# shroglck/open-pi-zero

Measured on AMD Instinct MI355X. Metric: train samples/sec at gbsz 1024 (bf16 fwd+bwd+clip+AdamW), higher is better.
Workload: dtype bf16; 1 GPU; Pi0 bridge training step: 256 img + 20 text + 1 proprio + 4 action tokens; model=pi0 (SigLIP-So400m/14 + Gemma-2B + 0.3B action expert), global_batch=1024, micro_batch=256, grad_accum=4, seq_len=281, parallelism=dp1

## Files before the change

open-pi-zero_amd/csrc/pz_flash.hip:

```cpp
#include "pz_common.h"

#include <type_traits>

namespace {

constexpr int FA_KB = 64;
constexpr int FA_NW = 4;
constexpr int FA_QS = 32;

template <int HD>
struct FaDims {
  static constexpr int HDK = (HD + 31) / 32 * 32;
  static constexpr int HDV = (HD + 15) / 16 * 16;
  static constexpr int NKS = HDK / 32;
  static constexpr int NDB = HDV / 16;
  static constexpr int ROW = HD == 256 ? 272 : (HD == 72 ? 112 : HDK + 16);
  static constexpr int FNW = HD == 256 ? 8 : 4;
  static constexpr int FNQB = HD == 256 ? 1 : 2;
};

__device__ __forceinline__ bool fa_allowed(int64_t i, int64_t j, int64_t cnt, int64_t P, int64_t C) {
  if (i < P) return i < cnt && j < cnt;
  if (i < P + C) return j < cnt || (j >= P && j < P + C);
  return j < cnt || j >= P;
// ... 697 lines not shown
    crow[qb] = mk.dead(t) ? 0.f : ff.crow_live;
  }
  f32x4 dq[D::NDB][2];
#pragma unroll
  for (int db = 0; db < D::NDB; ++db) dq[db][0] = dq[db][1] = f32x4{0.f, 0.f, 0.f, 0.f};

  __syncthreads();
  stk.store(Ks2[0]);
  stv.store(Vs2[0]);
  __syncthreads();
  for (int kb = 0; kb < nkb; ++kb) {
    const bf16_t* Ks = Ks2[kb & 1];
    const bf16_t* Vs = Vs2[kb & 1];
    const bool more = kb + 1 < nkb;
    if (more) {
      stk.load(K, a.ldk, (int64_t)(kb + 1) * JQ_KB, a.nk);
      stv.load(V, a.ldv, (int64_t)(kb + 1) * JQ_KB, a.nk);
    }
    const bool full = (kb + 1) * JQ_KB <= full_keys;
    f32x4 ds[2][2];
#pragma unroll
    for (int i = 0; i < 2; ++i) {
      bf16x8 kfr[D::NKS], vfr[D::NKS];
#pragma unroll
      for (int ks = 0; ks < D::NKS; ++ks) {
        kfr[ks] = frag_row<D::ROW>(Ks, i * 16, ks * 32, lane);
        vfr[ks] = frag_row<D::ROW>(Vs, i * 16, ks * 32, lane);
      }
#pragma unroll
      for (int qb = 0; qb < 2; ++qb) {
        f32x4 sv = {0.f, 0.f, 0.f, 0.f}, dp = {0.f, 0.f, 0.f, 0.f};
#pragma unroll
        for (int ks = 0; ks < D::NKS; ++ks) {
          sv = mfma(kfr[ks], qf[qb][ks], sv);
          dp = mfma(vfr[ks], df[qb][ks], dp);
        }
#pragma unroll
        for (int e = 0; e < 4; ++e) {
          const bool ok = full || ((rb[qb] >> fa_key_class(mk, kb * JQ_KB + i * 16 + 4 * g + e)) & 1);
          float pe, dse;
          ff.eval<CAP>(sv[e], dp[e], lse2[qb], crow[qb], del[qb], ok, pe, dse);
          ds[i][qb][e] = dse;
        }
      }
    }
    const bf16x8 sb0 = pack8(ds[0][0], ds[1][0]), sb1 = pack8(ds[0][1], ds[1][1]);
    constexpr int HB = (D::NDB + 1) / 2;
#pragma unroll
    for (int hb = 0; hb < 2; ++hb) {
      bf16x8 kt[HB];
#pragma unroll
      for (int x = 0; x < HB; ++x)
        if (hb * HB + x < D::NDB) kt[x] = frag_tr<D::ROW>(Ks, 0, (hb * HB + x) * 16, lane);
#pragma unroll
      for (int x = 0; x < HB; ++x) {
        const int db = hb * HB + x;
        if (db < D::NDB) {
          dq[db][0] = mfma(kt[x], sb0, dq[db][0]);
          dq[db][1] = mfma(kt[x], sb1, dq[db][1]);
        }
      }
    }
    if (more) {
      stk.store(Ks2[(kb + 1) & 1]);
      stv.store(Vs2[(kb + 1) & 1]);
    }
    __syncthreads();
  }
#pragma unroll
  for (int qb = 0; qb < 2; ++qb) {
    const int64_t r = (int64_t)qblk * RPW + wave * 32 + qb * 16 + (lane & 15);
    if (r >= a.nq) continue;
    bf16_t* dQ = (bf16_t*)a.dq + b * a.q_bstride + h * a.q_hstride + r * a.ldq;
#pragma unroll
    for (int db = 0; db < D::NDB; ++db) {
      const int d = db * 16 + 4 * g;
      if (d < HD)
        *reinterpret_cast<u32x2*>(dQ + d) = u32x2{pack2bf(dq[db][qb][0] * ff.scale, dq[db][qb][1] * ff.scale),
                                                  pack2bf(dq[db][qb][2] * ff.scale, dq[db][qb][3] * ff.scale)};
    }
  }
}

constexpr int JP_NW = 8, JP_MAXKB = 5;

constexpr int FR_MAX = 256, FR_NW = 8;

template <int HD>
__global__ void __launch_bounds__(FR_NW * 64) flash_fwd_res_kernel(pz_flash_args a) {
  using D = FaDims<HD>;
  constexpr int NT = FR_NW * 64;
  extern __shared__ __attribute__((aligned(16))) char fa_smem[];
  bf16_t* Kall = reinterpret_cast<bf16_t*>(fa_smem);
  bf16_t* Vall = Kall + FR_MAX * D::ROW;
  const int lane = threadIdx.x & 63, wave = threadIdx.x >> 6, g = lane >> 4;
  int64_t zh;
  int qblk;
  fa_unit_block((int)((a.nq + FR_NW * 16 - 1) / (FR_NW * 16)), (int)(a.Z * a.H), zh, qblk);
  const int64_t b = zh / a.H, h = zh % a.H;
  const int64_t q0 = (int64_t)qblk * (FR_NW * 16) + wave * 16;
  const bf16_t* Q = (const bf16_t*)a.q + b * a.q_bstride + h * a.q_hstride;
  const bf16_t* K = (const bf16_t*)a.k + b * a.k_bstride + h * a.k_hstride;
  const bf16_t* V = (const bf16_t*)a.v + b * a.v_bstride + h * a.v_hstride;
  const FaMask mk(a, b);
  {
    TileStager<HD, D::ROW, FR_MAX, NT> stk, stv;
    stk.load(K, a.ldk, 0, a.nk);
    stv.load(V, a.ldv, 0, a.nk);
    zero_pad_cols<HD, D::HDK, D::ROW, FR_MAX, NT>(Kall);
    zero_pad_cols<HD, D::HDK, D::ROW, FR_MAX, NT>(Vall);
    stk.store(Kall);
    stv.store(Vall);
  }
  bf16x8 qf[D::NKS];
  const int64_t rq = q0 + (lane & 15);
#pragma unroll
  for (int ks = 0; ks < D::NKS; ++ks) {
    const int c = ks * 32 + 8 * g;
    qf[ks] = (rq < a.nq && c < HD) ? *reinterpret_cast<const bf16x8*>(Q + rq * a.ldq + c) : bf16x8{};
  }
  f32x4 o[D::NDB];
#pragma unroll
  for (int db = 0; db < D::NDB; ++db) o[db] = f32x4{0.f, 0.f, 0.f, 0.f};
  float m = -INFINITY, l = 0.f;
  const int t = mk.token((int)rq);
  const int nkb = (int)((a.nk + FA_KB - 1) / FA_KB);
  __syncthreads();
  for (int kb = 0; kb < nkb; ++kb) {
    const bf16_t* Ks = Kall + kb * FA_KB * D::ROW;
    const bf16_t* Vs = Vall + kb * FA_KB * D::ROW;
    f32x4 sc[4];
#pragma unroll
    for (int i = 0; i < 4; ++i) sc[i] = f32x4{0.f, 0.f, 0.f, 0.f};
#pragma unroll
    for (int ks = 0; ks < D::NKS; ++ks)
#pragma unroll
      for (int i = 0; i < 4; ++i) sc[i] = mfma(frag_row<D::ROW>(Ks, i * 16, ks * 32, lane), qf[ks], sc[i]);
    float mx = -INFINITY;
#pragma unroll
    for (int i = 0; i < 4; ++i)
#pragma unroll
      for (int e = 0; e < 4; ++e) {
        const float x = fa_logit(mk, sc[i][e], t, kb * FA_KB + i * 16 + 4 * g + e);
        sc[i][e] = x;
        mx = fmaxf(mx, x);
      }
    mx = fmaxf(mx, __shfl_xor(mx, 16, 64));
    mx = fmaxf(mx, __shfl_xor(mx, 32, 64));
    const float mn = fmaxf(m, mx);
    const float alpha = mn == -INFINITY ? 1.f : __expf(m - mn);
    float sum = 0.f;
#pragma unroll
    for (int i = 0; i < 4; ++i)
#pragma unroll
      for (int e = 0; e < 4; ++e) {
        const float pv = mn == -INFINITY ? 0.f : __expf(sc[i][e] - mn);
        sc[i][e] = pv;
        sum += pv;
      }
    sum += __shfl_xor(sum, 16, 64);
    sum += __shfl_xor(sum, 32, 64);
    l = l * alpha + sum;
    m = mn;
#pragma unroll
    for (int db = 0; db < D::NDB; ++db) o[db] *= alpha;
    const bf16x8 pf0 = pack8(sc[0], sc[1]), pf1 = pack8(sc[2], sc[3]);
#pragma unroll
// ... 1206 lines not shown
          f32x4 sv = {0.f, 0.f, 0.f, 0.f}, dp = {0.f, 0.f, 0.f, 0.f};
#pragma unroll
          for (int ks = 0; ks < 3; ++ks) {
            sv = mfma(qa[ks], kfr[kb2][ks], sv);
            dp = mfma(da[ks], vfr[kb2][ks], dp);
          }
          float pe[4], de[4];
#pragma unroll
          for (int e = 0; e < 4; ++e) {
            pe[e] = __builtin_amdgcn_exp2f(fmaf(sv[e], sl2, -l2r[e]));
            de[e] = pe[e] * (dp[e] - dlr[e]);
          }
          pp[i][kb2][0] = pack2bf(pe[0], pe[1]);
          pp[i][kb2][1] = pack2bf(pe[2], pe[3]);
          dd[i][kb2][0] = pack2bf(de[0], de[1]);
          dd[i][kb2][1] = pack2bf(de[2], de[3]);
        }
      }
      if (last && un < units) issue_kv(un);
      auto cat4 = [](unsigned x0, unsigned x1, unsigned x2, unsigned x3) {
        return __builtin_bit_cast(bf16x8, u32x4{x0, x1, x2, x3});
      };
      const bf16x8 pb0 = cat4(pp[0][0][0], pp[0][0][1], pp[1][0][0], pp[1][0][1]);
      const bf16x8 pb1 = cat4(pp[0][1][0], pp[0][1][1], pp[1][1][0], pp[1][1][1]);
      const bf16x8 sb0 = cat4(dd[0][0][0], dd[0][0][1], dd[1][0][0], dd[1][0][1]);
      const bf16x8 sb1 = cat4(dd[0][1][0], dd[0][1][1], dd[1][1][0], dd[1][1][1]);
      const unsigned da0 = fs_lds_addr(Ds + (4 * g + ((lane & 15) >> 2)) * FS_ROW + 4 * (lane & 3));
      const unsigned qa0 = fs_lds_addr(Qs + (4 * g + ((lane & 15) >> 2)) * FS_ROW + 4 * (lane & 3));
      s16x4 td[5][2], tq[5][2];
#define FS_TR(db, hf)                                             \
  td[db][hf] = fs_tr<(16 * (hf)) * FS_ROW * 2 + (db) * 32>(da0); \
  tq[db][hf] = fs_tr<(16 * (hf)) * FS_ROW * 2 + (db) * 32>(qa0)
#define FS_MM(db)                                                                \
  {                                                                              \
    const bf16x8 dt = fs_cat(td[db][0], td[db][1]), qt = fs_cat(tq[db][0], tq[db][1]); \
    dv[db][0] = mfma(dt, pb0, dv[db][0]);                                        \
    dv[db][1] = mfma(dt, pb1, dv[db][1]);                                        \
    dk[db][0] = mfma(qt, sb0, dk[db][0]);                                        \
    dk[db][1] = mfma(qt, sb1, dk[db][1]);                                        \
  }
      FS_TR(0, 0); FS_TR(0, 1); FS_TR(1, 0); FS_TR(1, 1);
      asm volatile("s_waitcnt lgkmcnt(0)"
                   : "+v"(td[0][0]), "+v"(td[0][1]), "+v"(td[1][0]), "+v"(td[1][1]), "+v"(tq[0][0]), "+v"(tq[0][1]),
                     "+v"(tq[1][0]), "+v"(tq[1][1]));
      FS_TR(2, 0); FS_TR(2, 1); FS_TR(3, 0); FS_TR(3, 1);
      FS_MM(0) FS_MM(1)
      asm volatile("s_waitcnt lgkmcnt(0)"
                   : "+v"(td[2][0]), "+v"(td[2][1]), "+v"(td[3][0]), "+v"(td[3][1]), "+v"(tq[2][0]), "+v"(tq[2][1]),
                     "+v"(tq[3][0]), "+v"(tq[3][1]));
      FS_TR(4, 0); FS_TR(4, 1);
      FS_MM(2) FS_MM(3)
      asm volatile("s_waitcnt lgkmcnt(0)" : "+v"(td[4][0]), "+v"(td[4][1]), "+v"(tq[4][0]), "+v"(tq[4][1]));
      FS_MM(4)
#undef FS_MM
#undef FS_TR
    };
#pragma unroll 1
    for (int qs = 0; qs < FS_N / FA_QS - 1; ++qs) step(qs, false);
    step(FS_N / FA_QS - 1, true);
    FS_WAIT_VM(0);
#pragma unroll
    for (int kb2 = 0; kb2 < 2; ++kb2) {
      const int key = wave * 32 + kb2 * 16 + (lane & 15);
      bf16_t* dK = (bf16_t*)a.dk + b * a.k_bstride + h * a.k_hstride + (int64_t)key * a.ldk;
      bf16_t* dV = (bf16_t*)a.dv + b * a.v_bstride + h * a.v_hstride + (int64_t)key * a.ldv;
#pragma unroll
      for (int db = 0; db < 5; ++db) {
        const int d = db * 16 + 4 * g;
        if (d < 72) {
          *reinterpret_cast<u32x2*>(dK + d) = u32x2{pack2bf(dk[db][kb2][0] * a.scale, dk[db][kb2][1] * a.scale),
                                                    pack2bf(dk[db][kb2][2] * a.scale, dk[db][kb2][3] * a.scale)};
          *reinterpret_cast<u32x2*>(dV + d) =
              u32x2{pack2bf(dv[db][kb2][0], dv[db][kb2][1]), pack2bf(dv[db][kb2][2], dv[db][kb2][3])};
        }
      }
    }
    if (un < units && w0) tix.publish(tk, fa_smem + ((t + 1) & 1) * 2 * FS_IMG + FS_SLOT1);
    FS_BARRIER();
    u = un;
  }
}

constexpr int JD_SLOT = 64 * 512, JD_SMEM = 4 * JD_SLOT;

struct JdDma {
  int wave, lane;
  bool trs;
  __device__ __forceinline__ JdDma(int wave_, int lane_, bool trs_) : wave(wave_), lane(lane_), trs(trs_) {}
  __device__ __forceinline__ void issue(const bf16_t* X, int64_t ld, int kb, int nk, char* slot, int) const {
    int ln = lane;
    asm volatile("" : "+v"(ln));
#pragma unroll
    for (int s = 0; s < 4; ++s) {
      const int r = 2 * (wave * 4 + s) + (ln >> 5), pch = ln & 31;
      const int coff = 8 * (pch ^ (trs ? 2 * (r & 7) : (r & 15)));
      int key = kb * 64 + r;
      key = key < nk ? key : nk - 1;
      fs_glds16(X + (int64_t)key * ld + coff, slot + (wave * 4 + s) * 1024);
    }
  }
};

template <int K2, int DG>
__device__ __forceinline__ void jd_pv_group(f32x4 (&o)[16], const unsigned (&vs)[8], const bf16x8& pk) {
  s16x4 tv[4][2];
#define JD_TR(u, hf) tv[u][hf] = fs_tr<(K2 * 32 + 16 * (hf)) * 512 + ((DG * 4 + (u)) & 8) * 32>(vs[(DG * 4 + (u)) & 7])
  JD_TR(0, 0); JD_TR(0, 1); JD_TR(1, 0); JD_TR(1, 1); JD_TR(2, 0); JD_TR(2, 1); JD_TR(3, 0); JD_TR(3, 1);
#undef JD_TR
  asm volatile("s_waitcnt lgkmcnt(0)"
               : "+v"(tv[0][0]), "+v"(tv[0][1]), "+v"(tv[1][0]), "+v"(tv[1][1]), "+v"(tv[2][0]), "+v"(tv[2][1]),
                 "+v"(tv[3][0]), "+v"(tv[3][1]));
#pragma unroll
  for (int u = 0; u < 4; ++u) o[DG * 4 + u] = mfma(fs_cat(tv[u][0], tv[u][1]), pk, o[DG * 4 + u]);
}

template <bool CAP>
__global__ void __launch_bounds__(JP_NW * 64, 1) flash_fwd_probs_dma_kernel(pz_flash_args a, bf16_t* P, bf16_t* TC,
                                                                         int64_t ldp) {
  extern __shared__ __attribute__((aligned(16))) char fa_smem[];
  constexpr int RPW = JP_NW * 16;
  const int lane = threadIdx.x & 63, wave = threadIdx.x >> 6, g = lane >> 4, l15 = lane & 15;
  int64_t zh;
  int qblk;
  fa_unit_block((int)((a.nq + RPW - 1) / RPW), (int)(a.Z * a.H), zh, qblk);
  const int64_t b = zh / a.H, h = zh % a.H;
  const int64_t r = (int64_t)qblk * RPW + wave * 16 + l15;
  const bool live = r < a.nq;
  const bf16_t* Q = (const bf16_t*)a.q + b * a.q_bstride + h * a.q_hstride;
  const bf16_t* K = (const bf16_t*)a.k + b * a.k_bstride + h * a.k_hstride;
  const bf16_t* V = (const bf16_t*)a.v + b * a.v_bstride + h * a.v_hstride;
  const FaMask mk(a, b);
  const FaFast ff(a);
  const int nk = (int)a.nk;
  const JdDma dmk(wave, lane, false), dmv(wave, lane, true);
  bf16x8 qf[8];
  {
    const bf16_t* qrow = Q + (live ? r : 0) * a.ldq + 8 * g;
#define JD_QLD(ks) asm volatile("global_load_dwordx4 %0, %1, off offset:%2" : "=v"(qf[ks]) : "v"(qrow), "i"((ks) * 64) : "memory")
    JD_QLD(0); JD_QLD(1); JD_QLD(2); JD_QLD(3); JD_QLD(4); JD_QLD(5); JD_QLD(6); JD_QLD(7);
#undef JD_QLD
  }
  auto issue = [&](int s) {
    char* slot = fa_smem + (s % 4) * JD_SLOT;
    if (s < 5) dmk.issue(K, a.ldk, s, nk, slot, wave);
    else dmv.issue(V, a.ldv, s - 5, nk, slot, wave);
  };
  issue(0);
  issue(1);
  issue(2);
  const int t = mk.token((int)r);
  const bool dead = mk.dead(t);
  const int rb = fa_row_bits(mk, t), full_keys = fa_full_keys(mk);
  const bool clean = __ballot(dead || !live) == 0ull;
  f32x4 sc[JP_MAXKB][4];
  u32x2 tcv[JP_MAXKB][4];
  float mx = -INFINITY;
  auto logits_blk = [&](int kb) {
    auto logits = [&](auto FAST) {
#pragma unroll
      for (int i = 0; i < 4; ++i) {
        float tv[4];
#pragma unroll
        for (int e = 0; e < 4; ++e) {
          const float sv = sc[kb][i][e];
          float th = 0.f, x2;
          if constexpr (CAP) {
            th = fmaf(-2.f, __builtin_amdgcn_rcpf(__builtin_amdgcn_exp2f(sv * ff.k2) + 1.f), 1.f);
            x2 = th * ff.crow_live;
          } else {
            x2 = sv * ff.crow_live;
          }
          if constexpr (!decltype(FAST)::value) {
            const int j = kb * FA_KB + i * 16 + 4 * g + e;
            const bool ok = j < nk && (j < full_keys || ((rb >> fa_key_class(mk, j)) & 1));
            x2 = ok ? x2 : -INFINITY;
            th = (dead || j >= nk) ? 0.f : th;
          }
          sc[kb][i][e] = x2;
          mx = fmaxf(mx, x2);
          tv[e] = th;
        }
        tcv[kb][i] = u32x2{pack2bf(tv[0], tv[1]), pack2bf(tv[2], tv[3])};
      }
    };
    if (clean && (kb + 1) * 64 <= full_keys) logits(std::true_type{});
    else logits(std::false_type{});
  };
#pragma unroll
  for (int kb = 0; kb < JP_MAXKB; ++kb) {
    FS_WAIT_VM(8);
    FS_BARRIER();
    if (kb == 0)
      asm volatile("" : "+v"(qf[0]), "+v"(qf[1]), "+v"(qf[2]), "+v"(qf[3]), "+v"(qf[4]), "+v"(qf[5]), "+v"(qf[6]),
                   "+v"(qf[7]));
    issue(kb + 3);
    const char* slot = fa_smem + (kb % 4) * JD_SLOT + l15 * 512;
#pragma unroll
    for (int i = 0; i < 4; ++i) sc[kb][i] = f32x4{0.f, 0.f, 0.f, 0.f};
#pragma unroll
    for (int ks = 0; ks < 8; ++ks) {
      const char* kp = slot + 16 * ((4 * ks + g) ^ l15);
#pragma unroll
      for (int i = 0; i < 4; ++i) sc[kb][i] = mfma(*reinterpret_cast<const bf16x8*>(kp + i * 8192), qf[ks], sc[kb][i]);
    }
    if (kb >= 1) logits_blk(kb - 1);
  }
  logits_blk(JP_MAXKB - 1);
  FS_WAIT_VM(4);
  bf16_t* prow = P + (b * a.nq + (live ? r : 0)) * ldp;
  if (TC) {
    bf16_t* trow = TC + (b * a.nq + (live ? r : 0)) * ldp;
#pragma unroll
    for (int kb = 0; kb < JP_MAXKB; ++kb)
#pragma unroll
      for (int i = 0; i < 4; ++i) {
        const int j0 = kb * FA_KB + i * 16 + 4 * g;
        if (clean && (kb + 1) * 64 <= full_keys) *reinterpret_cast<u32x2*>(trow + j0) = tcv[kb][i];
// ... 2 lines not shown
  }
  mx = fs_max4(mx);
  float sum = 0.f;
#pragma unroll
  for (int kb = 0; kb < JP_MAXKB; ++kb)
#pragma unroll
    for (int i = 0; i < 4; ++i)
#pragma unroll
      for (int e = 0; e < 4; ++e) {
        const float pv = __builtin_amdgcn_exp2f(sc[kb][i][e] - mx);
        sc[kb][i][e] = pv;
        sum += pv;
      }
  sum = fs_sum4(sum);
  const float inv = 1.f / sum, uni = 1.f / (float)nk;
  bf16x8 pf[JP_MAXKB][2];
#pragma unroll
  for (int kb = 0; kb < JP_MAXKB; ++kb) {
    unsigned pk[4][2];
    auto probs = [&](auto FAST) {
#pragma unroll
      for (int i = 0; i < 4; ++i) {
        if constexpr (decltype(FAST)::value) {
          pk[i][0] = pack2bf(sc[kb][i][0] * inv, sc[kb][i][1] * inv);
          pk[i][1] = pack2bf(sc[kb][i][2] * inv, sc[kb][i][3] * inv);
        } else {
          float pv[4];
#pragma unroll
          for (int e = 0; e < 4; ++e) {
            const int j = kb * FA_KB + i * 16 + 4 * g + e;
            pv[e] = dead ? (j < nk ? uni : 0.f) : sc[kb][i][e] * inv;
          }
          pk[i][0] = pack2bf(pv[0], pv[1]);
          pk[i][1] = pack2bf(pv[2], pv[3]);
        }
        const int j0 = kb * FA_KB + i * 16 + 4 * g;
        if (decltype(FAST)::value || (live && j0 < ldp)) *reinterpret_cast<u32x2*>(prow + j0) = u32x2{pk[i][0], pk[i][1]};
      }
    };
    if (clean && (kb + 1) * 64 <= full_keys) probs(std::true_type{});
    else probs(std::false_type{});
    pf[kb][0] = __builtin_bit_cast(bf16x8, u32x4{pk[0][0], pk[0][1], pk[1][0], pk[1][1]});
    pf[kb][1] = __builtin_bit_cast(bf16x8, u32x4{pk[2][0], pk[2][1], pk[3][0], pk[3][1]});
  }
  f32x4 o[16];
#pragma unroll
  for (int db = 0; db < 16; ++db) o[db] = f32x4{0.f, 0.f, 0.f, 0.f};
  const int q4 = l15 >> 2, p4 = lane & 3, w = 4 * (g & 1) + q4;
  unsigned va[8];
#pragma unroll
  for (int d7 = 0; d7 < 8; ++d7) va[d7] = fs_lds_addr(fa_smem + (4 * g + q4) * 512 + 32 * (d7 ^ w) + 8 * p4);
#pragma unroll
  for (int kb = 0; kb < JP_MAXKB; ++kb) {
    const int s = 5 + kb;
    if (s == 7) FS_WAIT_VM(8);
    if (s == 8) FS_WAIT_VM(4);
    if (s == 9) FS_WAIT_VM(0);
    FS_BARRIER();
    if (s + 3 <= 9) issue(s + 3);
    const unsigned sb = (unsigned)((s % 4) * JD_SLOT);
    unsigned vs[8];
#pragma unroll
    for (int d7 = 0; d7 < 8; ++d7) vs[d7] = va[d7] + sb;
    jd_pv_group<0, 0>(o, vs, pf[kb][0]);
    jd_pv_group<0, 1>(o, vs, pf[kb][0]);
    jd_pv_group<0, 2>(o, vs, pf[kb][0]);
    jd_pv_group<0, 3>(o, vs, pf[kb][0]);
    jd_pv_group<1, 0>(o, vs, pf[kb][1]);
    jd_pv_group<1, 1>(o, vs, pf[kb][1]);
    jd_pv_group<1, 2>(o, vs, pf[kb][1]);
    jd_pv_group<1, 3>(o, vs, pf[kb][1]);
  }
  if (!live) return;
  const FaRow fr{&a};
  const int gi = fr.grp(r);
  bf16_t* O = (bf16_t*)a.g_o[gi] + fr.off(b, h, r, gi);
#pragma unroll
  for (int db = 0; db < 16; ++db) {
    const int d = db * 16 + 4 * g;
    *reinterpret_cast<u32x2*>(O + d) = u32x2{pack2bf(o[db][0], o[db][1]), pack2bf(o[db][2], o[db][3])};
  }
}

__global__ void __launch_bounds__(JP_NW * 64, 1) flash_bwd_ds_dma_kernel(pz_flash_args a, const bf16_t* P,
                                                                      const bf16_t* TC, bf16_t* dS, int64_t ldp) {
  extern __shared__ __attribute__((aligned(16))) char fa_smem[];
  constexpr int RPW = JP_NW * 16;
  const int lane = threadIdx.x & 63, wave = threadIdx.x >> 6, g = lane >> 4, l15 = lane & 15;
  int64_t zh;
  int qblk;
  fa_unit_block((int)((a.nq + RPW - 1) / RPW), (int)(a.Z * a.H), zh, qblk);
  const int64_t b = zh / a.H, h = zh % a.H;
  const int64_t r = (int64_t)qblk * RPW + wave * 16 + l15;
  const bool live = r < a.nq;
  const bool want_dq = a.dq != nullptr;
  const bf16_t* V = (const bf16_t*)a.v + b * a.v_bstride + h * a.v_hstride;
  const bf16_t* K = want_dq ? (const bf16_t*)a.k + b * a.k_bstride + h * a.k_hstride : V;
  const int64_t ldk = want_dq ? a.ldk : a.ldv;
  const int nk = (int)a.nk;
  const JdDma dmv(wave, lane, false), dmk(wave, lane, true);
  auto issue = [&](int s) {
    char* slot = fa_smem + (s % 4) * JD_SLOT;
    if (s < 5) dmv.issue(V, a.ldv, s, nk, slot, wave);
    else dmk.issue(K, ldk, s - 5, nk, slot, wave);
  };
  bf16x8 df[8];
  bool has_do;
  {
    const FaRow fr{&a};
    const int gi = live ? fr.grp(r) : 0;
    has_do = live && a.g_do[gi];
    const bf16_t* dOr = has_do ? (const bf16_t*)a.g_do[gi] + fr.off(b, h, r, gi) + 8 * g : V;
#define JD_DLD(ks) asm volatile("global_load_dwordx4 %0, %1, off offset:%2" : "=v"(df[ks]) : "v"(dOr), "i"((ks) * 64) : "memory")
    JD_DLD(0); JD_DLD(1); JD_DLD(2); JD_DLD(3); JD_DLD(4); JD_DLD(5); JD_DLD(6); JD_DLD(7);
#undef JD_DLD
  }
  issue(0);
  issue(1);
  issue(2);
  const bf16_t* prow = P + (b * a.nq + (live ? r : 0)) * ldp;
  const bf16_t* trow = TC ? TC + (b * a.nq + (live ? r : 0)) * ldp : prow;
  const bool clean = __ballot(!live) == 0ull;
  f32x4 dp[JP_MAXKB][4];
  u32x2 pw[JP_MAXKB][4], tw[JP_MAXKB][4];
#pragma unroll
  for (int kb = 0; kb < JP_MAXKB; ++kb) {
    FS_WAIT_VM(8);
    FS_BARRIER();
    if (kb == 0) {
      asm volatile("" : "+v"(df[0]), "+v"(df[1]), "+v"(df[2]), "+v"(df[3]), "+v"(df[4]), "+v"(df[5]), "+v"(df[6]),
                   "+v"(df[7]));
      if (!has_do) {
#pragma unroll
        for (int ks = 0; ks < 8; ++ks) df[ks] = bf16x8{};
      }
    }
    issue(kb + 3);
    const char* slot = fa_smem + (kb % 4) * JD_SLOT + l15 * 512;
#pragma unroll
    for (int i = 0; i < 4; ++i) dp[kb][i] = f32x4{0.f, 0.f, 0.f, 0.f};
#pragma unroll
    for (int ks = 0; ks < 8; ++ks) {
      const char* vp = slot + 16 * ((4 * ks + g) ^ l15);
#pragma unroll
      for (int i = 0; i < 4; ++i) dp[kb][i] = mfma(*reinterpret_cast<const bf16x8*>(vp + i * 8192), df[ks], dp[kb][i]);
    }
  }
  int gl = g;
  asm volatile("" : "+v"(gl));
#pragma unroll
  for (int k2 = 0; k2 < JP_MAXKB; ++k2)
#pragma unroll
    for (int i = 0; i < 4; ++i) {
      const int j0 = k2 * FA_KB + i * 16 + 4 * gl;
      const int jc = j0 < ldp ? j0 : 0;
      asm volatile("global_load_dwordx2 %0, %1, off" : "=v"(pw[k2][i]) : "v"(prow + jc) : "memory");
    }
#pragma unroll
  for (int k2 = 0; k2 < JP_MAXKB; ++k2)
#pragma unroll
    for (int i = 0; i < 4; ++i) {
      const int j0 = k2 * FA_KB + i * 16 + 4 * gl;
      const int jc = j0 < ldp ? j0 : 0;
      asm volatile("global_load_dwordx2 %0, %1, off" : "=v"(tw[k2][i]) : "v"(trow + jc) : "memory");
    }
  FS_WAIT_VM(20);
  bf16_t* orow = dS + (b * a.nq + (live ? r : 0)) * ldp;
  const bool cap = a.cap > 0.f;
  float dot = 0.f;
#pragma unroll
  for (int kb = 0; kb < JP_MAXKB; ++kb)
#pragma unroll
    for (int i = 0; i < 4; ++i) {
      asm volatile("" : "+v"(pw[kb][i]));
      const int j0 = kb * FA_KB + i * 16 + 4 * g;
      if (!(live && j0 < nk)) pw[kb][i] = u32x2{0u, 0u};
      const float p0 = __uint_as_float(pw[kb][i][0] << 16), p1 = __uint_as_float(pw[kb][i][0] & 0xffff0000u);
      const float p2 = __uint_as_float(pw[kb][i][1] << 16), p3 = __uint_as_float(pw[kb][i][1] & 0xffff0000u);
      dot += p0 * dp[kb][i][0] + p1 * dp[kb][i][1] + p2 * dp[kb][i][2] + p3 * dp[kb][i][3];
    }
  dot += __shfl_xor(dot, 16, 64);
  dot += __shfl_xor(dot, 32, 64);
  FS_WAIT_VM(0);
#pragma unroll
  for (int kb = 0; kb < JP_MAXKB; ++kb)
#pragma unroll
    for (int i = 0; i < 4; ++i) asm volatile("" : "+v"(tw[kb][i]));
  bf16x8 dsf[JP_MAXKB][2];
#pragma unroll
  for (int kb = 0; kb < JP_MAXKB; ++kb) {
    unsigned pk[4][2];
#pragma unroll
    for (int i = 0; i < 4; ++i) {
      const int j0 = kb * FA_KB + i * 16 + 4 * g;
      const u32x2 tv2 = (cap && live && j0 < nk) ? tw[kb][i] : u32x2{0u, 0u};
      const float pv[4] = {__uint_as_float(pw[kb][i][0] << 16), __uint_as_float(pw[kb][i][0] & 0xffff0000u),
                           __uint_as_float(pw[kb][i][1] << 16), __uint_as_float(pw[kb][i][1] & 0xffff0000u)};
      const float tv[4] = {__uint_as_float(tv2[0] << 16), __uint_as_float(tv2[0] & 0xffff0000u),
                           __uint_as_float(tv2[1] << 16), __uint_as_float(tv2[1] & 0xffff0000u)};
      float x[4];
#pragma unroll
      for (int e = 0; e < 4; ++e) {
        x[e] = pv[e] * (dp[kb][i][e] - dot) * a.scale;
        if (cap) x[e] *= fmaf(-tv[e], tv[e], 1.f);
      }
      pk[i][0] = pack2bf(x[0], x[1]);
      pk[i][1] = pack2bf(x[2], x[3]);
      if (clean ? j0 < ldp : (live && j0 < ldp)) *reinterpret_cast<u32x2*>(orow + j0) = u32x2{pk[i][0], pk[i][1]};
    }
    dsf[kb][0] = __builtin_bit_cast(bf16x8, u32x4{pk[0][0], pk[0][1], pk[1][0], pk[1][1]});
    dsf[kb][1] = __builtin_bit_cast(bf16x8, u32x4{pk[2][0], pk[2][1], pk[3][0], pk[3][1]});
  }
  f32x4 dq[16];
#pragma unroll
  for (int db = 0; db < 16; ++db) dq[db] = f32x4{0.f, 0.f, 0.f, 0.f};
  const int q4 = l15 >> 2, p4 = lane & 3, w = 4 * (g & 1) + q4;
  unsigned ka[8];
#pragma unroll
  for (int d7 = 0; d7 < 8; ++d7) ka[d7] = fs_lds_addr(fa_smem + (4 * g + q4) * 512 + 32 * (d7 ^ w) + 8 * p4);
#pragma unroll
  for (int kb = 0; kb < JP_MAXKB; ++kb) {
    const int s = 5 + kb;
    if (s == 8) FS_WAIT_VM(4);
    if (s == 9) FS_WAIT_VM(0);
    FS_BARRIER();
    if (s + 3 <= 9) issue(s + 3);
    if (want_dq) {
      const unsigned sb = (unsigned)((s % 4) * JD_SLOT);
      unsigned ks_[8];
#pragma unroll
      for (int d7 = 0; d7 < 8; ++d7) ks_[d7] = ka[d7] + sb;
      jd_pv_group<0, 0>(dq, ks_, dsf[kb][0]);
      jd_pv_group<0, 1>(dq, ks_, dsf[kb][0]);
      jd_pv_group<0, 2>(dq, ks_, dsf[kb][0]);
      jd_pv_group<0, 3>(dq, ks_, dsf[kb][0]);
      jd_pv_group<1, 0>(dq, ks_, dsf[kb][1]);
      jd_pv_group<1, 1>(dq, ks_, dsf[kb][1]);
      jd_pv_group<1, 2>(dq, ks_, dsf[kb][1]);
      jd_pv_group<1, 3>(dq, ks_, dsf[kb][1]);
    }
  }
  if (!live || !want_dq) return;
  bf16_t* dQ = (bf16_t*)a.dq + b * a.q_bstride + h * a.q_hstride + r * a.ldq;
#pragma unroll
  for (int db = 0; db < 16; ++db) {
    const int d = db * 16 + 4 * g;
    *reinterpret_cast<u32x2*>(dQ + d) = u32x2{pack2bf(dq[db][0], dq[db][1]), pack2bf(dq[db][2], dq[db][3])};
  }
}

constexpr int F8_KB = 128, F8_KT = F8_KB * 256, F8_VT = 256 * F8_KB;
constexpr int F8_SMEM = 2 * (F8_KT + F8_VT) + 2 * F8_KB * 4;

__device__ __forceinline__ int f8_kswz(int r) { return (r & 3) | ((r >> 5) << 2); }
__device__ __forceinline__ int f8_vswz(int d) { return (d & 6) | ((d >> 3) & 1); }
__device__ __forceinline__ i32x8 f8_cat(const u32x4& lo, const u32x4& hi) {
  return i32x8{(int)lo[0], (int)lo[1], (int)lo[2], (int)lo[3], (int)hi[0], (int)hi[1], (int)hi[2], (int)hi[3]};
}
__device__ __forceinline__ unsigned f8_enc4(float a, float b, float c, float d) {
  int v = __builtin_amdgcn_cvt_pk_fp8_f32(a, b, 0, false);
  v = __builtin_amdgcn_cvt_pk_fp8_f32(c, d, v, true);
  return (unsigned)v;
}

__global__ void __launch_bounds__(512) flash_fwd_f8_kernel(pz_flash_args a, const uint8_t* __restrict__ qc,
                                                          const float* __restrict__ qs, const uint8_t* __restrict__ kc,
                                                          const float* __restrict__ ks, int64_t krows,
                                                          const uint8_t* __restrict__ vtc,
                                                          const float* __restrict__ vs, int64_t ldvt) {
  extern __shared__ __attribute__((aligned(16))) char fa_smem[];
  auto Kt = [&](int bi) { return fa_smem + bi * F8_KT; };
  auto Vt = [&](int bi) { return fa_smem + 2 * F8_KT + bi * F8_VT; };
  auto Sk = [&](int bi) { return reinterpret_cast<float*>(fa_smem + 2 * (F8_KT + F8_VT)) + bi * F8_KB; };
  const int t = threadIdx.x, lane = t & 63, wave = t >> 6, g = lane >> 4, l15 = lane & 15;
  const int64_t b = blockIdx.y;
  const int64_t q0 = (int64_t)blockIdx.x * 128 + wave * 16;
  const int64_t r = q0 + l15;
  const FaMask mk(a, b);
  const int nkb = (int)((a.nk + F8_KB - 1) / F8_KB);
  const int per = (nkb + (int)gridDim.z - 1) / (int)gridDim.z;
  const int kb_begin = (int)blockIdx.z * per, kb_end = min(nkb, kb_begin + per);
  u32x4 sk_[4], sv_[4];
  float sks = 0.f;
  auto load = [&](int kb) {
#pragma unroll
    for (int j = 0; j < 4; ++j) {
      const int c = t + 512 * j;
      const int64_t kr = min((int64_t)kb * F8_KB + (c >> 4), krows - 1);
      sk_[j] = *reinterpret_cast<const u32x4*>(kc + (b * krows + kr) * 256 + (c & 15) * 16);
      sv_[j] = *reinterpret_cast<const u32x4*>(vtc + (b * 256 + (c >> 3)) * ldvt + (int64_t)kb * F8_KB + (c & 7) * 16);
    }
    if (t < F8_KB) sks = ks[b * krows + min((int64_t)kb * F8_KB + t, krows - 1)];
  };
  auto store = [&](int bi) {
#pragma unroll
    for (int j = 0; j < 4; ++j) {
      const int c = t + 512 * j;
      const int kr = c >> 4, d = c >> 3;
      *reinterpret_cast<u32x4*>(Kt(bi) + kr * 256 + (((c & 15) ^ f8_kswz(kr)) << 4)) = sk_[j];
      *reinterpret_cast<u32x4*>(Vt(bi) + d * 128 + (((c & 7) ^ f8_vswz(d)) << 4)) = sv_[j];
    }
    if (t < F8_KB) Sk(bi)[t] = sks;
  };
  i32x8 qf[2];
  float sq = 0.f;
  {
    const bool ok = r < a.nq;
    const uint8_t* qr = qc + (b * a.nq + (ok ? r : 0)) * 256 + 32 * g;
#pragma unroll
    for (int k2 = 0; k2 < 2; ++k2) {
      const u32x4 lo = ok ? *reinterpret_cast<const u32x4*>(qr + 128 * k2) : u32x4{0u, 0u, 0u, 0u};
// ... 215 lines not shown
        static bool attr4 = false;
        fa_smem_attr(flash_fwd_sig_kernel<1>, FS_SMEM, attr4);
        hipLaunchKernelGGL(flash_fwd_sig_kernel<1>, dim3((unsigned)G), dim3(16 * 64), FS_SMEM, st, *a, G);
      }
    } else if (fa_plain(a)) {
      fa_smem_attr(flash_fwd_unit_kernel<72, true>, FR_SMEM_KQ, attr);
      hipLaunchKernelGGL((flash_fwd_unit_kernel<72, true>), gu, dim3(FU_NW * 64), FR_SMEM_KQ, st, *a);
    } else {
      fa_smem_attr(flash_fwd_unit_kernel<72, false>, FR_SMEM_KQ, attr2);
      hipLaunchKernelGGL((flash_fwd_unit_kernel<72, false>), gu, dim3(FU_NW * 64), FR_SMEM_KQ, st, *a);
    }
    PZ_CHECK_LAUNCH();
    return PZ_OK;
  }
  if (sp == 1 && fa_resident(a)) {
    static bool attr = false;
    fa_smem_attr(flash_fwd_res_kernel<72>, FR_SMEM_KQ, attr);
    hipLaunchKernelGGL(flash_fwd_res_kernel<72>, dim3((unsigned)((a->nq + FR_NW * 16 - 1) / (FR_NW * 16) * a->Z * a->H)),
                       dim3(FR_NW * 64), FR_SMEM_KQ, st, *a);
    PZ_CHECK_LAUNCH();
    return PZ_OK;
  }
  FA_DISPATCH(a->head_dim, flash_fwd_kernel, grid, dim3((a->head_dim == 256 ? 8 : 4) * 64), 0, st, *a);
  PZ_CHECK_LAUNCH();
  if (sp > 1) {
    const int64_t n = a->Z * a->H * a->nq * (a->head_dim / 4);
    FA_DISPATCH(a->head_dim, flash_fwd_combine_kernel, dim3((unsigned)((n + 255) / 256)), dim3(256), 0, st, *a,
                (int)sp);
    PZ_CHECK_LAUNCH();
  }
  return PZ_OK;
}


extern "C" int pz_flash_fwd_probs(const pz_flash_args* a, void* P, void* tcap, int64_t ldp, void* stream) {
  PZ_CHECK_ARG(a && a->q && a->k && a->v && P && a->Z > 0 && a->H > 0 && a->nq > 0 && a->nk > 0,
               "flash_fwd_probs: bad args");
  PZ_CHECK_ARG(a->head_dim == 256, "flash_fwd_probs: head_dim %lld (256 only)", (long long)a->head_dim);
  PZ_CHECK_ARG(a->nk <= JP_MAXKB * FA_KB && ldp >= a->nk && ldp % 4 == 0, "flash_fwd_probs: nk %lld / ldp %lld",
               (long long)a->nk, (long long)ldp);
  PZ_CHECK_ARG(a->mask_mode == 0 || (a->mask_mode == 1 && a->cnt && a->rows_per_token > 0),
               "flash_fwd_probs: mask mode %d", a->mask_mode);
  PZ_CHECK_ARG(a->n_groups >= 1 && a->n_groups <= 3 && a->g_row0[0] == 0, "flash_fwd_probs: output groups");
  for (int i = 0; i < a->n_groups; ++i) PZ_CHECK_ARG(a->g_o[i] && a->g_ld[i] % 4 == 0, "flash_fwd_probs: group %d", i);
  PZ_CHECK_ARG(PZ_ALIGNED(a->q, 16) && PZ_ALIGNED(a->k, 16) && PZ_ALIGNED(a->v, 16) && PZ_ALIGNED(P, 8) &&
                   (!tcap || PZ_ALIGNED(tcap, 8)) && a->ldq % 8 == 0 && a->ldk % 8 == 0 && a->ldv % 8 == 0 &&
                   a->q_bstride % 8 == 0 && a->k_bstride % 8 == 0 && a->v_bstride % 8 == 0,
               "flash_fwd_probs: operands need 16-byte aligned rows");
  PZ_CHECK_ARG(a->nq + a->mask_row0 < (1 << 22) && a->Z * a->H < 65536, "flash_fwd_probs: nq / units too large");
  const int64_t units = a->Z * a->H, nqb = (a->nq + JP_NW * 16 - 1) / (JP_NW * 16);
  {
    static bool attr0 = false, attr1 = false;
    if (a->cap > 0.f) {
      fa_smem_attr(flash_fwd_probs_dma_kernel<true>, JD_SMEM, attr1);
      hipLaunchKernelGGL(flash_fwd_probs_dma_kernel<true>, dim3((unsigned)(nqb * units)), dim3(JP_NW * 64), JD_SMEM,
                         (hipStream_t)stream, *a, (bf16_t*)P, (bf16_t*)tcap, ldp);
    } else {
      fa_smem_attr(flash_fwd_probs_dma_kernel<false>, JD_SMEM, attr0);
      hipLaunchKernelGGL(flash_fwd_probs_dma_kernel<false>, dim3((unsigned)(nqb * units)), dim3(JP_NW * 64), JD_SMEM,
                         (hipStream_t)stream, *a, (bf16_t*)P, (bf16_t*)tcap, ldp);
    }
    PZ_CHECK_LAUNCH();
    return PZ_OK;
  }
}

extern "C" int pz_flash_bwd_ds(const pz_flash_args* a, const void* P, const void* tcap, void* dS, int64_t ldp,
                               void* stream) {
  PZ_CHECK_ARG(a && a->v && P && dS && a->Z > 0 && a->H > 0 && a->nq > 0 && a->nk > 0, "flash_bwd_ds: bad args");
  PZ_CHECK_ARG(a->head_dim == 256, "flash_bwd_ds: head_dim %lld (256 only)", (long long)a->head_dim);
  PZ_CHECK_ARG(a->nk <= JP_MAXKB * FA_KB && ldp >= a->nk && ldp % 4 == 0, "flash_bwd_ds: nk %lld / ldp %lld",
               (long long)a->nk, (long long)ldp);
  PZ_CHECK_ARG(a->cap <= 0.f || tcap, "flash_bwd_ds: soft-cap needs tcap");
  PZ_CHECK_ARG(a->n_groups >= 1 && a->n_groups <= 3 && a->g_row0[0] == 0, "flash_bwd_ds: output groups");
  for (int i = 0; i < a->n_groups; ++i) PZ_CHECK_ARG(!a->g_do[i] || a->g_ld[i] % 8 == 0, "flash_bwd_ds: dO group %d", i);
  PZ_CHECK_ARG(PZ_ALIGNED(a->v, 16) && a->ldv % 8 == 0 && a->v_bstride % 8 == 0 && PZ_ALIGNED(P, 8) &&
                   PZ_ALIGNED(dS, 8) && (!tcap || PZ_ALIGNED(tcap, 8)),
               "flash_bwd_ds: alignment");
  if (a->dq)
    PZ_CHECK_ARG(a->k && PZ_ALIGNED(a->k, 16) && a->ldk % 8 == 0 && a->k_bstride % 8 == 0 && PZ_ALIGNED(a->dq, 8) &&
                     a->ldq % 4 == 0 && a->q_bstride % 4 == 0,
                 "flash_bwd_ds: dQ needs K (16-byte rows) and an 8-byte aligned dQ");
  PZ_CHECK_ARG(a->Z * a->H < 65536, "flash_bwd_ds: too many units");
  const int64_t units = a->Z * a->H, nqb = (a->nq + JP_NW * 16 - 1) / (JP_NW * 16);
  static bool attr = false;
  fa_smem_attr(flash_bwd_ds_dma_kernel, JD_SMEM, attr);
  hipLaunchKernelGGL(flash_bwd_ds_dma_kernel, dim3((unsigned)(nqb * units)), dim3(JP_NW * 64), JD_SMEM,
                     (hipStream_t)stream, *a, (const bf16_t*)P, (const bf16_t*)tcap, (bf16_t*)dS, ldp);
  PZ_CHECK_LAUNCH();
  return PZ_OK;
}

extern "C" int pz_flash_bwd_prep(const pz_flash_args* a, void* stream) {
  PZ_CHECK_ARG(a && a->delta && a->n_groups >= 1 && a->n_groups <= 3, "flash_bwd_prep: bad args");
  for (int i = 0; i < a->n_groups; ++i) PZ_CHECK_ARG(a->g_o[i] && a->g_do[i], "flash_bwd_prep: group %d", i);
  const int64_t rows = a->Z * a->H * a->nq;
  PZ_CHECK_ARG(fa_hd_ok(a->head_dim), "flash_bwd_prep: head_dim");
  FA_DISPATCH(a->head_dim, flash_bwd_prep_kernel, dim3((unsigned)((rows + 3) / 4)), dim3(256), 0, (hipStream_t)stream,
              *a);
  PZ_CHECK_LAUNCH();
  return PZ_OK;
}

extern "C" int pz_flash_bwd(const pz_flash_args* a, void* stream) {
  PZ_CHECK_ARG(a && a->lse && a->delta && a->dq && a->dk && a->dv, "flash_bwd: bad args");
  PZ_CHECK_ARG(fa_hd_ok(a->head_dim), "flash_bwd: head_dim");
  PZ_CHECK_ARG(PZ_ALIGNED(a->dq, 16) && PZ_ALIGNED(a->dk, 16) && PZ_ALIGNED(a->dv, 16), "flash_bwd: alignment");
  for (int i = 0; i < a->n_groups; ++i) PZ_CHECK_ARG(a->g_do[i] && a->g_ld[i] % 8 == 0, "flash_bwd: dO group %d", i);
  hipStream_t st = (hipStream_t)stream;
  const int64_t nkb = (a->nk + FA_KB - 1) / FA_KB;
  int64_t splits = 1;
  if (a->ws && a->head_dim % 4 == 0) {
    splits = (1024 + nkb * a->Z * a->H - 1) / (nkb * a->Z * a->H);
    splits = splits < 8 ? splits : 8;
    while (splits > 1 && splits * 2 * a->Z * a->H * a->nk * a->head_dim * 4 > a->ws_bytes) --splits;
  }
  if (fa_resident(a) && fa_unit(a)) {
    static bool aq = false, akv = false, aq2 = false, akv2 = false, aq3 = false, akv3 = false;
    const dim3 gu((unsigned)(a->Z * a->H));
    if (fa_sig(a)) {
      const int G = fa_sig_grid(a);
      fa_smem_attr(flash_bwd_kv_sig_kernel, FS_SMEM, akv3);
      (void)aq3;
      {
        static bool aq4 = false;
        fa_smem_attr(flash_bwd_q_sig_kernel<true>, FS_SMEM, aq4);
        hipLaunchKernelGGL(flash_bwd_q_sig_kernel<true>, dim3((unsigned)G), dim3(FS_NW * 64), FS_SMEM, st, *a, G);
      }
      PZ_CHECK_LAUNCH();
      hipLaunchKernelGGL(flash_bwd_kv_sig_kernel, dim3((unsigned)G), dim3(FS_NW * 64), FS_SMEM, st, *a, G);
    } else if (fa_plain(a)) {
      fa_smem_attr(flash_bwd_q_unit_kernel<72, true>, FR_SMEM_KQ, aq);
      fa_smem_attr(flash_bwd_kv_unit_kernel<72, true>, FU_SMEM_KV, akv);
      hipLaunchKernelGGL((flash_bwd_q_unit_kernel<72, true>), gu, dim3(FU_NW * 64), FR_SMEM_KQ, st, *a);
      PZ_CHECK_LAUNCH();
      hipLaunchKernelGGL((flash_bwd_kv_unit_kernel<72, true>), gu, dim3(FU_NW * 64), FU_SMEM_KV, st, *a);
    } else {
      fa_smem_attr(flash_bwd_q_unit_kernel<72, false>, FR_SMEM_KQ, aq2);
      fa_smem_attr(flash_bwd_kv_unit_kernel<72, false>, FU_SMEM_KV, akv2);
      hipLaunchKernelGGL((flash_bwd_q_unit_kernel<72, false>), gu, dim3(FU_NW * 64), FR_SMEM_KQ, st, *a);
      PZ_CHECK_LAUNCH();
      hipLaunchKernelGGL((flash_bwd_kv_unit_kernel<72, false>), gu, dim3(FU_NW * 64), FU_SMEM_KV, st, *a);
    }
    PZ_CHECK_LAUNCH();
    return PZ_OK;
  }
  if (fa_resident(a)) {
    static bool aq = false, akv = false;
    fa_smem_attr(flash_bwd_q_res_kernel<72>, FR_SMEM_KQ, aq);
    fa_smem_attr(flash_bwd_kv_res_kernel<72>, FR_SMEM_KV, akv);
    hipLaunchKernelGGL(flash_bwd_q_res_kernel<72>, dim3((unsigned)((a->nq + FR_NW * 16 - 1) / (FR_NW * 16) * a->Z * a->H)),
                       dim3(FR_NW * 64), FR_SMEM_KQ, st, *a);
    PZ_CHECK_LAUNCH();
    hipLaunchKernelGGL(flash_bwd_kv_res_kernel<72>, dim3((unsigned)(nkb * a->Z * a->H)), dim3(FR_NW * 64),
                       FR_SMEM_KV, st, *a);
    PZ_CHECK_LAUNCH();
    return PZ_OK;
  }
  const int fm = fa_fast_bwd(a);
  {
    const int64_t units = a->Z * a->H, nqb = (a->nq + JQ_NW * 32 - 1) / (JQ_NW * 32);
    const dim3 gq2((unsigned)(nqb * units));
    if (fm == 2) {
      FA_DISPATCH(a->head_dim, FA_T2(flash_bwd_q2_kernel, true), gq2, dim3(JQ_NW * 64), 0, st, *a);
    } else {
      FA_DISPATCH(a->head_dim, FA_T2(flash_bwd_q2_kernel, false), gq2, dim3(JQ_NW * 64), 0, st, *a);
    }
  }
  PZ_CHECK_LAUNCH();
  const dim3 gkv1((unsigned)(nkb * a->Z * a->H * splits));
// ... 53 lines not shown
```

Before: 273.8 samples/s.

## Shrink flash dS backward workgroups to four waves with double-buffered DMA

The dS backward kernel now uses 4-wave workgroups covering 64 rows each instead of 8 waves, and two shared-memory slots instead of four. This halves LDS per workgroup so two workgroups fit per CU, with launch bounds raised to match. The DMA helper is templated on wave count so each wave issues more loads. Prefetch depth falls from three stages to one, with full vmcnt waits, which may expose load latency. K/V tiles are also reloaded for twice as many row blocks.

```diff
diff --git a/open-pi-zero_amd/csrc/pz_flash.hip b/open-pi-zero_amd/csrc/pz_flash.hip
--- a/open-pi-zero_amd/csrc/pz_flash.hip
+++ b/open-pi-zero_amd/csrc/pz_flash.hip
@@ -803,7 +803,7 @@
   }
 }
 
-constexpr int JP_NW = 8, JP_MAXKB = 5;
+constexpr int JP_NW = 8, JS_NW = 4, JP_MAXKB = 5;
 
 constexpr int FR_MAX = 256, FR_NW = 8;
 
@@ -2176,8 +2176,13 @@
 }
 
 constexpr int JD_SLOT = 64 * 512, JD_SMEM = 4 * JD_SLOT;
-
+constexpr int JS_SMEM = 2 * JD_SLOT;
+static_assert(2 * JS_SMEM <= 160 * 1024, "two dS workgroups per CU");
+
+template <int NW>
 struct JdDma {
+  static constexpr int PER = JD_SLOT / 1024 / NW;
+  static_assert(PER * NW * 1024 == JD_SLOT, "waves must divide the block's 32 DMA instructions");
   int wave, lane;
   bool trs;
   __device__ __forceinline__ JdDma(int wave_, int lane_, bool trs_) : wave(wave_), lane(lane_), trs(trs_) {}
@@ -2185,12 +2190,12 @@
     int ln = lane;
     asm volatile("" : "+v"(ln));
 #pragma unroll
-    for (int s = 0; s < 4; ++s) {
-      const int r = 2 * (wave * 4 + s) + (ln >> 5), pch = ln & 31;
+    for (int s = 0; s < PER; ++s) {
+      const int r = 2 * (wave * PER + s) + (ln >> 5), pch = ln & 31;
       const int coff = 8 * (pch ^ (trs ? 2 * (r & 7) : (r & 15)));
       int key = kb * 64 + r;
       key = key < nk ? key : nk - 1;
-      fs_glds16(X + (int64_t)key * ld + coff, slot + (wave * 4 + s) * 1024);
+      fs_glds16(X + (int64_t)key * ld + coff, slot + (wave * PER + s) * 1024);
     }
   }
 };
@@ -2226,7 +2231,7 @@
   const FaMask mk(a, b);
   const FaFast ff(a);
   const int nk = (int)a.nk;
-  const JdDma dmk(wave, lane, false), dmv(wave, lane, true);
+  const JdDma<JP_NW> dmk(wave, lane, false), dmv(wave, lane, true);
   bf16x8 qf[8];
   {
     const bf16_t* qrow = Q + (live ? r : 0) * a.ldq + 8 * g;
@@ -2395,10 +2400,10 @@
   }
 }
 
-__global__ void __launch_bounds__(JP_NW * 64, 1) flash_bwd_ds_dma_kernel(pz_flash_args a, const bf16_t* P,
+__global__ void __launch_bounds__(JS_NW * 64, 2) flash_bwd_ds_dma_kernel(pz_flash_args a, const bf16_t* P,
                                                                       const bf16_t* TC, bf16_t* dS, int64_t ldp) {
   extern __shared__ __attribute__((aligned(16))) char fa_smem[];
-  constexpr int RPW = JP_NW * 16;
+  constexpr int RPW = JS_NW * 16;
   const int lane = threadIdx.x & 63, wave = threadIdx.x >> 6, g = lane >> 4, l15 = lane & 15;
   int64_t zh;
   int qblk;
@@ -2411,9 +2416,9 @@
   const bf16_t* K = want_dq ? (const bf16_t*)a.k + b * a.k_bstride + h * a.k_hstride : V;
   const int64_t ldk = want_dq ? a.ldk : a.ldv;
   const int nk = (int)a.nk;
-  const JdDma dmv(wave, lane, false), dmk(wave, lane, true);
+  const JdDma<JS_NW> dmv(wave, lane, false), dmk(wave, lane, true);
   auto issue = [&](int s) {
-    char* slot = fa_smem + (s % 4) * JD_SLOT;
+    char* slot = fa_smem + (s % 2) * JD_SLOT;
     if (s < 5) dmv.issue(V, a.ldv, s, nk, slot, wave);
     else dmk.issue(K, ldk, s - 5, nk, slot, wave);
   };
@@ -2430,7 +2435,6 @@
   }
   issue(0);
   issue(1);
-  issue(2);
   const bf16_t* prow = P + (b * a.nq + (live ? r : 0)) * ldp;
   const bf16_t* trow = TC ? TC + (b * a.nq + (live ? r : 0)) * ldp : prow;
   const bool clean = __ballot(!live) == 0ull;
@@ -2438,7 +2442,8 @@
   u32x2 pw[JP_MAXKB][4], tw[JP_MAXKB][4];
 #pragma unroll
   for (int kb = 0; kb < JP_MAXKB; ++kb) {
-    FS_WAIT_VM(8);
+    if (kb == 0) FS_WAIT_VM(8);
+    else FS_WAIT_VM(0);
     FS_BARRIER();
     if (kb == 0) {
       asm volatile("" : "+v"(df[0]), "+v"(df[1]), "+v"(df[2]), "+v"(df[3]), "+v"(df[4]), "+v"(df[5]), "+v"(df[6]),
@@ -2448,8 +2453,8 @@
         for (int ks = 0; ks < 8; ++ks) df[ks] = bf16x8{};
       }
     }
-    issue(kb + 3);
-    const char* slot = fa_smem + (kb % 4) * JD_SLOT + l15 * 512;
+    if (kb >= 1) issue(kb + 1);
+    const char* slot = fa_smem + (kb % 2) * JD_SLOT + l15 * 512;
 #pragma unroll
     for (int i = 0; i < 4; ++i) dp[kb][i] = f32x4{0.f, 0.f, 0.f, 0.f};
 #pragma unroll
@@ -2534,12 +2539,11 @@
 #pragma unroll
   for (int kb = 0; kb < JP_MAXKB; ++kb) {
     const int s = 5 + kb;
-    if (s == 8) FS_WAIT_VM(4);
-    if (s == 9) FS_WAIT_VM(0);
+    if (s >= 6) FS_WAIT_VM(0);
     FS_BARRIER();
-    if (s + 3 <= 9) issue(s + 3);
+    if (s + 1 <= 9) issue(s + 1);
     if (want_dq) {
-      const unsigned sb = (unsigned)((s % 4) * JD_SLOT);
+      const unsigned sb = (unsigned)((s % 2) * JD_SLOT);
       unsigned ks_[8];
 #pragma unroll
       for (int d7 = 0; d7 < 8; ++d7) ks_[d7] = ka[d7] + sb;
@@ -2921,10 +2925,11 @@
                      a->ldq % 4 == 0 && a->q_bstride % 4 == 0,
                  "flash_bwd_ds: dQ needs K (16-byte rows) and an 8-byte aligned dQ");
   PZ_CHECK_ARG(a->Z * a->H < 65536, "flash_bwd_ds: too many units");
-  const int64_t units = a->Z * a->H, nqb = (a->nq + JP_NW * 16 - 1) / (JP_NW * 16);
+  const int64_t units = a->Z * a->H, nqb = (a->nq + JS_NW * 16 - 1) / (JS_NW * 16);
+  PZ_CHECK_ARG(nqb * units < (1ll << 31), "flash_bwd_ds: too many row blocks");
   static bool attr = false;
-  fa_smem_attr(flash_bwd_ds_dma_kernel, JD_SMEM, attr);
-  hipLaunchKernelGGL(flash_bwd_ds_dma_kernel, dim3((unsigned)(nqb * units)), dim3(JP_NW * 64), JD_SMEM,
+  fa_smem_attr(flash_bwd_ds_dma_kernel, JS_SMEM, attr);
+  hipLaunchKernelGGL(flash_bwd_ds_dma_kernel, dim3((unsigned)(nqb * units)), dim3(JS_NW * 64), JS_SMEM,
                      (hipStream_t)stream, *a, (const bf16_t*)P, (const bf16_t*)tcap, (bf16_t*)dS, ldp);
   PZ_CHECK_LAUNCH();
   return PZ_OK;
```

After: 274.1 samples/s (median of 6 runs). No clear change (+0.1%).
